# zhvng/open-musiclm

Measured on AMD Instinct MI355X. Metric: train steps/sec + AR tokens/sec, coarse-stage musiclm_small, higher is better.
Workload: dtype fp16ff; 1 GPU; musiclm_small coarse-stage train step (fwd+bwd+allreduce+clip+AdamW), N=1116 (3 start + 13 clap + 200 semantic + 900 coarse), forgetful mask 0.15, ff_dropout 0.1; global_batch=32, per_gpu_batch=32, grad_accum=1, seq_len=1116, parallelism=dp1, precision=fp16ff, hip_graph=True, exchange=none (single GPU)

## Files before the change

### include/omlm.h

```cpp
#ifndef OMLM_H
#define OMLM_H
#include <stdint.h>
#ifdef __cplusplus
extern "C" {
#endif

int         omlm_version(void);
const char* omlm_last_error(void);
void        omlm_set_error(const char* msg);

int omlm_gemm(const void* A, const void* B, void* C, const float* Cin,
              const int* a_map, const int* b_map, const int* c_map, long long a_rows, long long b_rows,
              int M, int N, int K, int lda, int ldb, int ldc, int ldcin,
              int a_kmajor, int b_kmajor, int in_dtype, int out_dtype, float alpha,
              void* workspace, long long workspace_bytes, void* stream);
long long omlm_gemm_tail_workspace_bytes(int M, int N);

int omlm_layernorm_fwd(const float* x, const float* gamma, void* y, void* xcast, float* mean, float* rstd,
                       int M, int D, int ldy, float eps, int out_dtype, void* stream);
int omlm_layernorm_fwd_planes(const float* x, const float* gamma, void* y, void* y_lo, float* mean, float* rstd,
                              int M, int D, int ldy, float eps, int out_dtype, void* stream);
int omlm_layernorm_fwd_seg(const float* x, const float* gamma, void* y, void* xcast, float* mean, float* rstd, float* xc,
                           int M, int D, int ldy, float eps, int out_dtype, int n_full, int p0, int n_live, void* stream);
int omlm_layernorm_fwd_planes_seg(const float* x, const float* gamma, void* y, void* y_lo, float* mean, float* rstd, float* xc,
                                  int M, int D, int ldy, float eps, int out_dtype, int n_full, int p0, int n_live, void* stream);
int omlm_layernorm_bwd2_seg(const void* dy, const float* x, const float* gamma, const float* mean, const float* rstd,
                            const float* dres, const void* dres2, float* dx, void* dxcast, float* dgamma, float* workspace, int M, int D,
                            float dx_scale, int cast_dtype, int dy_dtype, int n_full, int p0, int n_live, void* stream);
long long omlm_layernorm_bwd_workspace_bytes(int D);
int omlm_layernorm_bwd2(const void* dy, const float* x, const float* gamma, const float* mean, const float* rstd,
                        const float* dres, const void* dres2, float* dx, void* dxcast, float* dgamma, float* workspace, int M, int D,
                        float dx_scale, int cast_dtype, int dy_dtype, void* stream);

int omlm_qk_norm_fwd(const float* q_raw, const float* kv_raw, const float* q_scale, const float* k_scale,
                     void* q, void* k, void* v, int M, int H, int out_dtype, void* stream);
int omlm_qk_norm_bwd(const float* dq, const float* dk, const float* dv, const float* q_raw, const float* kv_raw,
                     const float* q_scale, const float* k_scale, void* dq_raw, void* dkv_raw,
                     float* dq_scale, float* dk_scale, int M, int H, int out_dtype, void* stream);

int omlm_gemm_qknorm(const void* A, const void* B, void* C, void* C2, int c2_col0, int ldc2, const float* scale, float* norm_out,
                     int ldnorm, int groups, long long a_rows, long long b_rows, int M, int N, int K, int lda, int ldb, int ldc,
                     int dtype, void* stream);
int omlm_qk_norm_bwd2(const float* dq, const float* dk, const float* dv, const void* q, const void* k, const float* qn, const float* kn,
                      const float* q_scale, const float* k_scale, void* dq_raw, void* dkv_raw, float* dq_scale, float* dk_scale,
                      int M, int H, int dtype, void* stream);

int omlm_mqa_attn_fwd(const void* q, const void* k, const void* v, const float* bias, const float* biasT, const unsigned char* keymask,
                      void* out, float* lse, int B, int N, int H, float scale, int bias_ld, int dtype, int P, float p,
                      unsigned long long seed, const unsigned long long* seed_dev, void* stream);
long long omlm_attn_bias_table_floats(int N, int H, int P);
int omlm_attn_bias_prepare(const float* bias, float* biasT, int N, int H, int bias_ld, const float* q_scale,
                           const float* k_scale, float qk_bound, float scale, int p_max_log2, void* stream);
int omlm_attn_bias_prepare_group(const float* bias, float* const* biasT, int layers, int N, int H, int bias_ld,
                                 const float* const* q_scale, const float* const* k_scale, float qk_bound, float scale,
                                 int p_max_log2, int P, void* stream);
int omlm_attn_max_positions(int dtype, int P);
long long omlm_mqa_attn_bwd_workspace_bytes(int B, int N, int H);
int omlm_mqa_attn_bwd(const void* q, const void* k, const void* v, const float* bias, const float* biasT, const unsigned char* keymask,
                      const void* out, const void* dout, const float* lse, float* delta, float* dq, float* dk, float* dv, float* dbias,
                      float* dbias_ws, int B, int N, int H, float scale, int bias_ld, int dtype, int P, float p, unsigned long long seed,
                      const unsigned long long* seed_dev, void* stream);
int omlm_attn_dropout_keep(unsigned char* keep, int B, int N, int H, float p, unsigned long long seed,
                           const unsigned long long* seed_dev, void* stream);
int omlm_dropout_residual_fwd(const float* x, const float* y, float* x1, long long M, int D, float p, unsigned long long seed,
                              const unsigned long long* seed_dev, void* stream);
int omlm_dropout_residual_bwd(const float* dx1, void* dy, long long M, int D, float p, unsigned long long seed,
                              const unsigned long long* seed_dev, int out_dtype, void* stream);

int omlm_ffmid_fwd(const void* h1, const void* convw, const void* gamma, void* h2, float* mean, float* rstd,
                   int M, int nseq, int F, int Fp, float eps, float p, unsigned long long seed,
                   const unsigned long long* seed_dev, unsigned char* drop_bits, void* gh, int dtype, void* stream);
int omlm_ffmid_fwd_planes(const void* h1, const void* h1_lo, const void* convw, const void* convw_lo, const void* gamma, const void* gamma_lo,
                          void* h2, void* h2_lo, float* mean, float* rstd, int M, int nseq, int F, int Fp, float eps, float p,
                          unsigned long long seed, const unsigned long long* seed_dev, unsigned char* drop_bits, void* gh, int dtype, void* stream);
int omlm_ffmid_fwd_seg(const void* h1, const void* convw, const void* gamma, void* h2, float* mean, float* rstd,
                       int M, int nseq, int F, int Fp, float eps, float p, unsigned long long seed,
                       const unsigned long long* seed_dev, unsigned char* drop_bits, void* gh, int dtype, int n_full, int p0, void* stream);
int omlm_ffmid_fwd_planes_seg(const void* h1, const void* h1_lo, const void* convw, const void* convw_lo, const void* gamma, const void* gamma_lo,
                              void* h2, void* h2_lo, float* mean, float* rstd, int M, int nseq, int F, int Fp, float eps, float p,
                              unsigned long long seed, const unsigned long long* seed_dev, unsigned char* drop_bits, void* gh, int dtype,
                              int n_full, int p0, void* stream);
long long omlm_ffmid_bwd_workspace_bytes(int F, int Fp);
int omlm_ffmid_bwd(const void* dh2, const void* h1, const void* convw, const void* gamma, const float* mean,
                   const float* rstd, void* du_tmp, void* dh1, float* dgamma, float* dconv, float* workspace,
                   int M, int nseq, int F, int Fp, float p, unsigned long long seed,
                   const unsigned long long* seed_dev, const unsigned char* drop_bits, const void* gh, int dtype, void* stream);
int omlm_colsum_accumulate(const float* part, float* out, int P, int C, int ldp, void* stream);
typedef struct omlm_colsum_desc { const float* part; float* out; int P, C, ldp; } omlm_colsum_desc;
int omlm_colsum_group(const omlm_colsum_desc* problems, int count, void* stream);
int omlm_ffmid_set_impl(int impl);

int omlm_embed_gather_fwd(const int* ids, const int* seg, const int* posidx,
                          const float* const* tables, const float* const* starts, const float* const* pos,
                          int nseq, float* out, int B, int N, int D,
                          const long long* table_rows, const long long* pos_rows, int* err_flag, void* stream);
int omlm_embed_gather_bwd(const int* ids, const int* seg, const int* posidx,
                          float* const* dtables, float* const* dstarts, float* const* dpos,
                          int nseq, const float* dx, int B, int N, int D, float alpha,
                          const long long* table_rows, const long long* pos_rows, int* err_flag, void* stream);

int omlm_prepare_train_batch(const long long* const* ids, int* const* labels, const int* len, const int* eos, const int* Q,
                             const int* codebook, int nseq, int B, int pad_id, const float* scores, int n_drop,
                             int* ids32, unsigned char* keymask, int N, const float* null_u, float null_p, void* stream);

int omlm_cross_entropy_fwd(const float* logits, const int* labels, float* row_lse, float* nll_sum,
                           int R, int V, int ld, int* err_flag, void* stream);
int omlm_cross_entropy_bwd(const float* logits, const int* labels, const float* row_lse, const float* gscale,
                           float coef, void* dlogits, int R, int V, int ld, int ldd, int out_dtype, void* stream);
int omlm_cross_entropy_fwd_reg(const float* logits, const int* labels, float* row_lse, float* sums,
                               int R, int V, int ld, int* err_flag, void* stream);
int omlm_cross_entropy_bwd_reg(const float* logits, const int* labels, const float* row_lse, const float* gscale,
                               float coef, void* dlogits, int R, int V, int ld, int ldd, int out_dtype,
                               float label_smoothing, float z_loss, void* stream);
int omlm_ce_metrics(const float* logits, const int* labels, float* row_nll, int* row_rank, float* row_entropy,
                    int R, int V, int ld, int* err_flag, void* stream);
// ... 177 lines not shown
```

### open_musiclm_amd/engine.py

```python
from __future__ import annotations

import math
import os
from dataclasses import dataclass, field
from typing import Dict, List, Optional, Sequence, Tuple

import torch

from . import ops
from .hip import require_gpu

ATTN_SCALE = 8.0
DIM_HEAD = 64

_PRECISIONS = {"bf16": torch.bfloat16, "bf16x3": torch.float32, "fp16": torch.float16, "fp16ff": torch.float16}


def is_half(precision: str) -> bool:
    return precision in ("fp16", "fp16ff")
_H16 = (torch.bfloat16, torch.float16)



FF_PLANES_MAX_FP = 4096
# ... 90 lines not shown

def build_layout(B: int, lens: Sequence[int], quantizers: Sequence[int], device, final_rows_only: bool = False) -> SeqLayout:
    starts, pos = [], 0
    for l in lens:
        starts.append(pos)
        pos += l + 1
    N = pos
    seg = torch.empty(N, dtype=torch.int32)
    posidx = torch.zeros(N, dtype=torch.int32)
    start_col = torch.zeros(N, dtype=torch.bool)
    for s, (st, l) in enumerate(zip(starts, lens)):
        seg[st: st + l + 1] = s
        start_col[st] = True
        posidx[st + 1: st + l + 1] = torch.arange(l, dtype=torch.int32)
    n_out = [l for l in lens[:-1]] + [lens[-1] + 1]
    lay = SeqLayout(B, N, tuple(lens), tuple(starts), tuple(n_out), seg.to(device), posidx.to(device),
                    start_col.to(device), final_rows_only)
    if final_rows_only:
        s, st, n_s, Q = len(lens) - 1, starts[-1], n_out[-1], quantizers[-1]
        b = torch.arange(B)
        a_map = (b * N + st + n_s - 1).to(torch.int32)
        lay.head_maps[(s, (n_s - 1) % Q)] = (a_map.to(device), b.to(torch.int32).to(device), B)
        return lay
    for s, (st, n_s, Q) in enumerate(zip(starts, n_out, quantizers)):
        for qq in range(Q):
            js = torch.arange(qq, n_s, Q)
            if js.numel() == 0:
                continue
            b = torch.arange(B)[:, None]
            a_map = (b * N + st + js[None, :]).reshape(-1).to(torch.int32)
            c_map = (b * n_s + js[None, :]).reshape(-1).to(torch.int32)
            lay.head_maps[(s, qq)] = (a_map.to(device), c_map.to(device), int(a_map.numel()))
    return lay


CONV_HALO = 2
LIVE_K_MULTIPLE = 64
FF_ONE_PASS_MAX_FP = 3072


def first_live_row(lay: SeqLayout, want: Sequence[bool]) -> Optional[int]:
    firsts = [st for st, n_s, w in zip(lay.starts, lay.n_out, want) if w and n_s > 0]
    return min(firsts) if firsts else None


def live_rows(lay: SeqLayout, want: Sequence[bool], B: int, T: torch.dtype, Fp: int, halo: int = CONV_HALO) -> Optional[Tuple[int, int, int]]:
    if os.environ.get("OMLM_LIVE_ROWS", "1") == "0":
        return None
    if lay.final_only or T == torch.float32 or Fp > FF_ONE_PASS_MAX_FP:
        return None
    first = first_live_row(lay, want)
    if first is None:
        return None
    N = lay.N
    g = LIVE_K_MULTIPLE // math.gcd(B, LIVE_K_MULTIPLE)
    top = first - halo
    if top < 0:
        return None
    p0 = top - (top - N) % g
    if p0 <= 0 or 16 * p0 < N:
        return None
    return N, p0, N - p0


def live_to_full(r, seg: Tuple[int, int, int]):
    n_full, p0, n_live = seg
    return (r // n_live) * n_full + p0 + r % n_live


def full_to_live(r, seg: Tuple[int, int, int]):
    n_full, p0, n_live = seg
    return (r // n_full) * n_live + r % n_full - p0


def head_map(lay: SeqLayout, s: int, qq: int, live: Optional[Tuple[int, int, int]]):
    ent = lay.head_maps.get((s, qq))
    if ent is None or live is None:
        return ent
    a_map, c_map, rows = ent
    key = (s, qq, live[1])
    if key not in lay.live_maps:
        lay.live_maps[key] = full_to_live(a_map, live).to(torch.int32)
    return lay.live_maps[key], c_map, rows


def h16_operand(w: torch.Tensor, T: torch.dtype) -> torch.Tensor:
    sh = getattr(w, "_omlm_bf16", None)
    if (sh is not None and sh.dtype == T and getattr(w, "_omlm_bf16_version", -1) == w._version and sh.device == w.device):
        return sh
    c = torch.empty(w.shape, dtype=T, device=w.device)
    ops.cast_pad(w.detach(), c, w.numel() // w.shape[-1], w.shape[-1], w.shape[-1], w.shape[-1])
    return c


class PreparedWeights:
    def __init__(self, model, precision: str, persistent: bool = True):
        tr = model.transformer
        self.precision = precision
        self.T = _PRECISIONS[precision]
        self.ff3 = precision == "fp16ff"
        T = self.T
        dev = model.start_tokens[0].device
        D = tr.dim
        Fp_all = {ceil_to(ff.inner_dim, 64) for _, _, ff in tr.layers}
        self.ff_planes = self.ff3 and all(ff_planes_ok(f) for f in Fp_all)
        self.mx = self.ff_planes and all(ff_mx_ok(D, f) for f in Fp_all)
        quants = ops.QuantRowsGroup()
        self.layers = []
        wbuf = model.__dict__.setdefault("_omlm_wbuf", {})
        packs = ops.CastPadGroup()
        for li, (attn, _, ff) in enumerate(tr.layers):
            F = ff.inner_dim
            Fp = ceil_to(F, 64)
            w1 = ff.w_in.weight
            w2 = ff.w_out.weight
            ent = {}
            if T == torch.float32:
                ent["Wq"], ent["Wkv"], ent["Wo"] = attn.to_q.weight, attn.to_kv.weight, attn.to_out[0].weight
            else:
                for name, w in (("Wq", attn.to_q.weight), ("Wkv", attn.to_kv.weight), ("Wo", attn.to_out[0].weight)):
                    ent[name] = h16_operand(w, T)
            bkey = (li, T, str(dev), F, D)
            if not persistent:
                W1p, W2p, convp, gammap = (torch.zeros(2 * Fp, D, dtype=T, device=dev), torch.zeros(D, Fp, dtype=T, device=dev),
                                           torch.zeros(3, 2 * Fp, dtype=T, device=dev), torch.zeros(Fp, dtype=T, device=dev))
            else:
                if bkey not in wbuf:
                    wbuf[bkey] = (torch.zeros(2 * Fp, D, dtype=T, device=dev), torch.zeros(D, Fp, dtype=T, device=dev),
                                  torch.zeros(3, 2 * Fp, dtype=T, device=dev), torch.zeros(Fp, dtype=T, device=dev))
                W1p, W2p, convp, gammap = wbuf[bkey]
            packs.add(w1.detach(), W1p, F, D, D, D)
            packs.add(w1.detach()[F:], W1p[Fp:], F, D, D, D)
            packs.add(w2.detach(), W2p, D, F, F, Fp)
            ent["W1p"], ent["W2p"], ent["F"], ent["Fp"] = W1p, W2p, F, Fp
            if self.ff_planes:
                lkey = bkey + ("lo",)
                if not persistent or lkey not in wbuf:
                    lo = (torch.zeros(2 * Fp, D, dtype=T, device=dev), torch.zeros(D, Fp, dtype=T, device=dev),
                          torch.zeros(3, 2 * Fp, dtype=T, device=dev), torch.zeros(Fp, dtype=T, device=dev))
                    if persistent:
                        wbuf[lkey] = lo
                else:
                    lo = wbuf[lkey]
                W1l, W2l, convl, gammal = lo
                if not (self.mx and persistent):
                    packs.add(w1.detach(), W1l, F, D, D, D, lo=True)
                    packs.add(w1.detach()[F:], W1l[Fp:], F, D, D, D, lo=True)
                    packs.add(w2.detach(), W2l, D, F, F, Fp, lo=True)
                ent["W1p_lo"], ent["W2p_lo"], ent["convw_lo"], ent["gamma_mid_lo"] = W1l, W2l, convl, gammal
            if self.mx:
                mkey = bkey + ("mx",)
                if not persistent or mkey not in wbuf:
                    m8 = (ops.Fp8Planes(2 * Fp, D, dev), ops.Fp8Planes(D, Fp, dev))
                    if persistent:
                        wbuf[mkey] = m8
                else:
                    m8 = wbuf[mkey]
                quants.add(w1.detach(), m8[0], 0, F, D, D)
                quants.add(w1.detach()[F:], m8[0], Fp, F, D, D)
                quants.add(w2.detach(), m8[1], 0, D, F, F)
                ent["W1p8"], ent["W2p8"] = m8
            cw = ff.conv_weight().detach().reshape(2 * F, 3)
            packs.add(cw, convp, F, 3, 3, 2 * Fp, transpose=True)
            packs.add(cw[F:], convp[:, Fp:], F, 3, 3, 2 * Fp, transpose=True)
            packs.add(ff.norm_mid.gamma.detach(), gammap, 1, F, F, Fp)
            ent["convw"], ent["gamma_mid"] = convp, gammap
# ... 153 lines not shown
    ops.gemm(dtable, lin[3].weight.detach(), dz, M=n, N=Hd, K=ldb, b_kmajor=True, lda=ldb, b_rows=H)
    for k in (2, 1):
        ds = torch.empty(n, Hd, device=dev)
        ops.silu_bwd(dz, pres[k], ds, n * Hd)
        ops.colsum_accumulate(ds, grad_of(lin[k].bias), n, Hd, Hd)
        gw = grad_of(lin[k].weight)
        ops.gemm(ds, zs[k - 1], gw, M=Hd, N=Hd, K=n, a_kmajor=True, b_kmajor=True, Cin=gw, planes=False)
        dz = torch.zeros(n, Hd, device=dev)
        ops.gemm(ds, lin[k].weight.detach(), dz, M=n, N=Hd, K=Hd, b_kmajor=True, Cin=dz, planes=False)
    ds = torch.empty(n, Hd, device=dev)
    ops.silu_bwd(dz, pres[0], ds, n * Hd)
    ops.colsum_accumulate(ds, grad_of(lin[0].bias), n, Hd, Hd)
    ops.relpos_first_bwd(ds, grad_of(lin[0].weight).view(-1), n, Hd, x0=x0)


class LayerSaved:
    __slots__ = ("x", "m1", "r1", "xn", "xc", "q_raw", "kv_raw", "q", "k", "v", "o", "lse", "abias",
                 "x1", "m2", "r2", "xn2", "h1", "h2", "m3", "r3", "seed", "p", "drop_bits", "gh", "h1_lo_tail",
                 "pa", "sa", "po", "so")


def _dropout_state(tr, dev):
    st = tr.__dict__.get("_omlm_dropout")
    if st is None or st["counter"].device != dev:
        rank = int(os.environ.get("RANK", "0"))
        g = torch.Generator().manual_seed((int(torch.initial_seed()) + 0x9E3779B1 * rank) & 0x7FFFFFFF)
        L = len(tr.layers)
        st = dict(counter=torch.zeros(1, dtype=torch.int64, device=dev),
                  seeds=[int(v) for v in torch.randint(1, 2 ** 62, (L,), generator=g)])
        a = [int(v) for v in torch.randint(1, 2 ** 62, (2 * L,), generator=g)]
        st["attn_seeds"], st["out_seeds"] = a[:L], a[L:]
        st["last"] = None
        tr.__dict__["_omlm_dropout"] = st
    return st


def dropout_salt(tr, dev) -> torch.Tensor:
    st = _dropout_state(tr, dev)
    st["counter"].add_(1)
    st["last"] = st["counter"].clone()
    return st["last"], st["seeds"]


def dropout_state(tr, dev=None) -> dict:
    st = tr.__dict__.get("_omlm_dropout")
    if st is None:
        st = _dropout_state(tr, dev if dev is not None else torch.device("cpu"))
    last = st["last"]
    return dict(ff=list(st["seeds"]), attn=list(st["attn_seeds"]), out=list(st["out_seeds"]),
                salt=int(last.item()) if last is not None else None)


def trunk_forward(tr, pw: PreparedWeights, x: torch.Tensor, keymask: Optional[torch.Tensor], B: int, N: int,
                  save: bool, training: bool, keep_h1_lo_tail: bool = False, live: Optional[Tuple[int, int, int]] = None):
    T = pw.T
    dev = x.device
    M, D = x.shape
    H = tr.heads
    P = prefix_rows(tr)
    rc = tr.__dict__.get("_omlm_relpos_cache")
    if rc is not None and save and training and rc.usable(N):
        table, rp_saved = rc.table, ("cached", rc)
    else:
        table, rp_saved = relpos_forward(tr, N, save, P)
        if (rc is not None and rc.enabled and rc.n is None and save and training and rp_saved is not None and rp_saved[0] != "t5"
                and not torch.cuda.is_current_stream_capturing()):
            rc.adopt(N, table, rp_saved)
            rp_saved = ("cached", rc)
    saved_layers: List[LayerSaved] = []
    abiases = None
    assert live is None or (len(tr.layers) > 0 and not keep_h1_lo_tail and live[0] == N)
    salt, seeds, aseeds, oseeds = (None, None, None, None)
    aps = [(float(a_.attn_dropout.p), float(a_.to_out[1].p)) if training else (0.0, 0.0) for a_, _, _ in tr.layers]
    if training and (any(float(ff.dropout_p) > 0 for _, _, ff in tr.layers) or any(pa > 0 or po > 0 for pa, po in aps)):
        salt, seeds = dropout_salt(tr, dev)
        st_ = tr.__dict__["_omlm_dropout"]
        aseeds, oseeds = st_["attn_seeds"], st_["out_seeds"]
    for li, ((attn, _, ff), w) in enumerate(zip(tr.layers, pw.layers)):
        sv = LayerSaved()
        F, Fp = w["F"], w["Fp"]
        m1 = torch.empty(M, device=dev); r1 = torch.empty(M, device=dev)
        xn = torch.empty(M, D, dtype=T, device=dev)
        xc = x if T == torch.float32 else torch.empty(M, D, dtype=T, device=dev)
        ops.layernorm_fwd(x, attn.norm.gamma.detach(), xn, None if T == torch.float32 else xc, m1, r1)
        q = torch.empty(M, H * DIM_HEAD, dtype=T, device=dev)
        k = torch.empty(M, DIM_HEAD, dtype=T, device=dev)
        v = torch.empty(M, DIM_HEAD, dtype=T, device=dev)
        fused_qk = T in _H16
        if fused_qk:
            qn = torch.empty(M, H, device=dev)
            kn = torch.empty(M, device=dev)
            q_raw, kv_raw = qn, kn
            ops.gemm_qknorm(xn, w["Wq"], q, attn.q_scale.detach(), qn, H, M=M, N=H * DIM_HEAD, K=D)
            ops.gemm_qknorm(xc, w["Wkv"], k, attn.k_scale.detach(), kn, 1, M=M, N=2 * DIM_HEAD, K=D, C2=v, c2_col0=DIM_HEAD)
        else:
            q_raw = torch.empty(M, H * DIM_HEAD, device=dev)
            kv_raw = torch.empty(M, 2 * DIM_HEAD, device=dev)
            ops.gemm(xn, w["Wq"], q_raw, M=M, N=H * DIM_HEAD, K=D)
            ops.gemm(xc, w["Wkv"], kv_raw, M=M, N=2 * DIM_HEAD, K=D)
            ops.qk_norm_fwd(q_raw, kv_raw, attn.q_scale.detach(), attn.k_scale.detach(), q, k, v, H)
        o = torch.empty(M, H * DIM_HEAD, dtype=T, device=dev)
        lse = torch.empty(B, H, N, device=dev)
        if abiases is None:
            abiases = ops.AttnBias.group(table, N, H, dev, [a_.q_scale.detach() for a_, _, _ in tr.layers],
                                         [a_.k_scale.detach() for a_, _, _ in tr.layers], scale=ATTN_SCALE, half=T == torch.float16, P=P)
        abias = abiases[li]
        pa, po = aps[li]
        sa = aseeds[li] if pa > 0 else 0
        so = oseeds[li] if po > 0 else 0
        ops.attn_fwd(q, k, v, abias, keymask, o, lse, B, N, H, ATTN_SCALE, P=P, p=pa, seed=sa, seed_dev=salt if pa > 0 else None)
        x1 = torch.empty(M, D, device=dev)
        if po > 0:
            yo = torch.empty(M, D, device=dev)
            ops.gemm(o, w["Wo"], yo, M=M, N=D, K=H * DIM_HEAD)
            ops.dropout_residual_fwd(x, yo, x1, po, so, seed_dev=salt)
            del yo
        else:
            ops.gemm(o, w["Wo"], x1, M=M, N=D, K=H * DIM_HEAD, Cin=x)
        seg = live if li == len(tr.layers) - 1 else None
        x1c = None
        if seg is not None:
            M = B * seg[2]
            nff = seg[2]
            x1c = torch.empty(M, D, device=dev)
        else:
            nff = N
        m2 = torch.empty(M, device=dev); r2 = torch.empty(M, device=dev)
        xn2 = torch.empty(M, D, dtype=T, device=dev)
        h1 = torch.empty(M, 2 * Fp, dtype=T, device=dev)
        if pw.mx:
            P1 = ops.Fp8Planes(M, D, dev, zero=False)
            ops.layernorm_fwd_mx(x1, ff.norm_in.gamma.detach(), xn2, P1, m2, r2, seg=seg, xc=x1c)
            h1_lo = torch.empty(M, 2 * Fp, dtype=torch.uint8, device=dev)
            ops.gemm_mx16(xn2, P1, w["W1p"], w["W1p8"], h1, h1_lo, M=M, N=2 * Fp, K=D)
        elif pw.ff_planes:
            xn2_lo = torch.empty(M, D, dtype=T, device=dev)
            ops.layernorm_fwd_planes(x1, ff.norm_in.gamma.detach(), xn2, xn2_lo, m2, r2, seg=seg, xc=x1c)
            h1_lo = torch.empty(M, 2 * Fp, dtype=T, device=dev)
            ops.gemm_planes16(xn2, xn2_lo, w["W1p"], w["W1p_lo"], h1, h1_lo, M=M, N=2 * Fp, K=D)
        else:
            ops.layernorm_fwd(x1, ff.norm_in.gamma.detach(), xn2, None, m2, r2, seg=seg, xc=x1c)
            ops.gemm(xn2, w["W1p"], h1, M=M, N=2 * Fp, K=D)
        if seg is not None:
            x1 = x1c
        h2 = torch.empty(M, Fp, dtype=T, device=dev)
        m3 = torch.empty(M, device=dev); r3 = torch.empty(M, device=dev)
        p = float(ff.dropout_p) if training else 0.0
        seed = seeds[li] if (p > 0 and seeds is not None) else 0
        drop_bits = torch.empty(M, Fp // 8, dtype=torch.uint8, device=dev) if (p > 0 and (save or pw.ff_planes)) else None
        gh = torch.empty(M, Fp, dtype=T, device=dev) if save else None
        x2 = torch.empty(M, D, device=dev)
        if pw.ff_planes:
            if pw.mx:
                P2 = ops.Fp8Planes(M, Fp, dev, zero=False)
                ops.ffmid_fwd_mx(h1, h1_lo, w["convw"], w["convw_lo"], w["gamma_mid"], w["gamma_mid_lo"], h2, P2, m3, r3, nff, F, Fp, p, seed,
                                 seed_dev=salt if p > 0 else None, drop_bits=drop_bits, gh=gh, seg=seg)
                ops.gemm_mx16(h2, P2, w["W2p"], w["W2p8"], x2, M=M, N=D, K=Fp, Cin=x1)
            else:
                h2_lo = torch.empty(M, Fp, dtype=T, device=dev)
                ops.ffmid_fwd_planes(h1, h1_lo, w["convw"], w["convw_lo"], w["gamma_mid"], w["gamma_mid_lo"], h2, h2_lo, m3, r3, nff, F, Fp, p, seed,
                                     seed_dev=salt if p > 0 else None, drop_bits=drop_bits, gh=gh, seg=seg)
                ops.gemm_planes16(h2, h2_lo, w["W2p"], w["W2p_lo"], x2, M=M, N=D, K=Fp, Cin=x1)
                del xn2_lo, h2_lo
            if keep_h1_lo_tail and save:
                take = min(2, N)
                sv.h1_lo_tail = torch.zeros(B, 2, 2 * Fp, device=dev)
                tail = h1_lo.view(B, N, -1)[:, N - take:]
                if tail.dtype == torch.uint8:
                    tail = (tail.contiguous().to(torch.int16) << 8).view(torch.float16)
                sv.h1_lo_tail[:, 2 - take:].copy_(tail)
            del h1_lo
        else:
            ops.ffmid_fwd(h1, w["convw"], w["gamma_mid"], h2, m3, r3, nff, F, Fp, p, seed, seed_dev=salt if p > 0 else None,
                          drop_bits=drop_bits, gh=gh, seg=seg)
            ops.gemm(h2, w["W2p"], x2, M=M, N=D, K=Fp, Cin=x1)
        if save:
            sv.x, sv.m1, sv.r1, sv.xn, sv.xc = x, m1, r1, xn, xc
# ... 409 lines not shown
```

### open_musiclm_amd/hip.py

```python
from __future__ import annotations

import ctypes as C
import os
from typing import Optional

import torch

_HERE = os.path.dirname(os.path.abspath(__file__))
LIB_PATH = os.environ.get("OMLM_LIB_PATH") or os.path.join(_HERE, "libomlm_hip.so")

_lib: Optional[C.CDLL] = None

vp, i32, i64, f32, u64, f64, u32 = C.c_void_p, C.c_int, C.c_longlong, C.c_float, C.c_ulonglong, C.c_double, C.c_uint

SIGNATURES = {
    "omlm_version": [],
    "omlm_last_error": [],
    "omlm_set_error": [C.c_char_p],
    "omlm_gemm": [vp, vp, vp, vp, vp, vp, vp, i64, i64, i32, i32, i32, i32, i32, i32, i32, i32, i32, i32, i32, f32, vp, i64, vp],
    "omlm_gemm_tail_workspace_bytes": [i32, i32],
    "omlm_gemm_wgrad_group": [vp, i32, i32, i32, vp],
    "omlm_gemm_planes": [vp, i64, vp, i64, vp, vp, vp, vp, vp, i64, i64, i32, i32, i32, i32, i32, i32, i32, i32, i32, i32, f32, vp, i64, vp],
    "omlm_split_planes": [vp, vp, i64, i64, vp],
    "omlm_gemm_planes16": [vp, vp, vp, vp, vp, vp, vp, vp, vp, i64, i64, i32, i32, i32, i32, i32, i32, i32, i32, vp, i64, vp],
    "omlm_gemm_mx16": [vp, vp, i64, vp, vp, vp, i64, vp, vp, vp, i32, vp, i64, i64, i32, i32, i32, i32, i32, i32, i32, vp, i64, vp],
    "omlm_gemm_mx16_workspace_bytes": [i32, i32, i32],
    "omlm_layernorm_fwd_mx": [vp, vp, vp, vp, i64, vp, vp, vp, i32, i32, i32, f32, vp],
    "omlm_ffmid_fwd_mx": [vp, vp, vp, vp, vp, vp, vp, vp, i64, vp, vp, vp, i32, i32, i32, i32, f32, f32, u64, vp, vp, vp, vp],
    "omlm_layernorm_fwd_mx_seg": [vp, vp, vp, vp, i64, vp, vp, vp, vp, i32, i32, i32, f32, i32, i32, i32, vp],
    "omlm_ffmid_fwd_mx_seg": [vp, vp, vp, vp, vp, vp, vp, vp, i64, vp, vp, vp, i32, i32, i32, i32, f32, f32, u64, vp, vp, vp, i32, i32, vp],
    "omlm_quant_rows_mx": [vp, i32, vp],
    "omlm_layernorm_fwd_planes": [vp, vp, vp, vp, vp, vp, i32, i32, i32, f32, i32, vp],
    "omlm_ffmid_fwd_planes": [vp, vp, vp, vp, vp, vp, vp, vp, vp, vp, i32, i32, i32, i32, f32, f32, u64, vp, vp, vp, i32, vp],
    "omlm_layernorm_fwd": [vp, vp, vp, vp, vp, vp, i32, i32, i32, f32, i32, vp],
    "omlm_layernorm_fwd_seg": [vp, vp, vp, vp, vp, vp, vp, i32, i32, i32, f32, i32, i32, i32, i32, vp],
    "omlm_layernorm_fwd_planes_seg": [vp, vp, vp, vp, vp, vp, vp, i32, i32, i32, f32, i32, i32, i32, i32, vp],
    "omlm_layernorm_bwd2_seg": [vp, vp, vp, vp, vp, vp, vp, vp, vp, vp, vp, i32, i32, f32, i32, i32, i32, i32, i32, vp],
    "omlm_layernorm_bwd_workspace_bytes": [i32],
    "omlm_layernorm_bwd2": [vp, vp, vp, vp, vp, vp, vp, vp, vp, vp, vp, i32, i32, f32, i32, i32, vp],
    "omlm_qk_norm_fwd": [vp, vp, vp, vp, vp, vp, vp, i32, i32, i32, vp],
    "omlm_qk_norm_bwd": [vp, vp, vp, vp, vp, vp, vp, vp, vp, vp, vp, i32, i32, i32, vp],
    "omlm_gemm_qknorm": [vp, vp, vp, vp, i32, i32, vp, vp, i32, i32, i64, i64, i32, i32, i32, i32, i32, i32, i32, vp],
    "omlm_qk_norm_bwd2": [vp, vp, vp, vp, vp, vp, vp, vp, vp, vp, vp, vp, vp, i32, i32, i32, vp],
    "omlm_attn_bias_table_floats": [i32, i32, i32],
    "omlm_attn_bias_prepare": [vp, vp, i32, i32, i32, vp, vp, f32, f32, i32, vp],
    "omlm_attn_bias_prepare_group": [vp, vp, i32, i32, i32, i32, vp, vp, f32, f32, i32, i32, vp],
    "omlm_mqa_attn_fwd": [vp] * 8 + [i32, i32, i32, f32, i32, i32, i32, f32, u64, vp, vp],
    "omlm_mqa_attn_bwd": [vp] * 15 + [i32, i32, i32, f32, i32, i32, i32, f32, u64, vp, vp],
    "omlm_mqa_attn_bwd_workspace_bytes": [i32, i32, i32],
    "omlm_attn_max_positions": [i32, i32],
    "omlm_attn_dropout_keep": [vp, i32, i32, i32, f32, u64, vp, vp],
    "omlm_dropout_residual_fwd": [vp, vp, vp, i64, i32, f32, u64, vp, vp],
    "omlm_dropout_residual_bwd": [vp, vp, i64, i32, f32, u64, vp, i32, vp],
    "omlm_ffmid_fwd": [vp, vp, vp, vp, vp, vp, i32, i32, i32, i32, f32, f32, u64, vp, vp, vp, i32, vp],
    "omlm_ffmid_fwd_seg": [vp, vp, vp, vp, vp, vp, i32, i32, i32, i32, f32, f32, u64, vp, vp, vp, i32, i32, i32, vp],
    "omlm_ffmid_fwd_planes_seg": [vp, vp, vp, vp, vp, vp, vp, vp, vp, vp, i32, i32, i32, i32, f32, f32, u64, vp, vp, vp, i32, i32, i32, vp],
    "omlm_ffmid_bwd_workspace_bytes": [i32, i32],
    "omlm_ffmid_bwd": [vp, vp, vp, vp, vp, vp, vp, vp, vp, vp, vp, i32, i32, i32, i32, f32, u64, vp, vp, vp, i32, vp],
    "omlm_colsum_accumulate": [vp, vp, i32, i32, i32, vp],
    "omlm_colsum_group": [vp, i32, vp],
    "omlm_ffmid_set_impl": [i32],
    "omlm_embed_gather_fwd": [vp, vp, vp, vp, vp, vp, i32, vp, i32, i32, i32, vp, vp, vp, vp],
    "omlm_embed_gather_bwd": [vp, vp, vp, vp, vp, vp, i32, vp, i32, i32, i32, f32, vp, vp, vp, vp],
    "omlm_prepare_train_batch": [vp, vp, vp, vp, vp, vp, i32, i32, i32, vp, i32, vp, vp, i32, vp, f32, vp],
    "omlm_cross_entropy_fwd": [vp, vp, vp, vp, i32, i32, i32, vp, vp],
    "omlm_cross_entropy_bwd": [vp, vp, vp, vp, f32, vp, i32, i32, i32, i32, i32, vp],
    "omlm_cross_entropy_fwd_reg": [vp, vp, vp, vp, i32, i32, i32, vp, vp],
    "omlm_cross_entropy_bwd_reg": [vp, vp, vp, vp, f32, vp, i32, i32, i32, i32, i32, f32, f32, vp],
    "omlm_ce_metrics": [vp, vp, vp, vp, vp, i32, i32, i32, vp, vp],
    "omlm_ce_metrics_bins": [vp, vp, vp, vp, i32, i32, i32, i32, i32, vp, vp],
    "omlm_sumsq_accumulate": [vp, i64, vp, vp, vp],
    "omlm_adamw_clip_step": [vp, vp, vp, vp, vp, i64, f32, f32, f32, f32, f32, i32, f32, vp, f32, i32, i32, i32, vp, vp],
    "omlm_adamw_clip_step_ema": [vp, vp, vp, vp, vp, i64, f32, f32, f32, f32, f32, i32, f32, vp, f32, i32, i32, i32, vp, vp, f32, i32, i32, vp],
    "omlm_loss_scale_update": [vp, vp, f32, f32, i32, f32, f32, vp],
    "omlm_cast_pad": [vp, vp, i64, i32, i32, i32, i32, vp],
    "omlm_cast_pad_group": [vp, i32, i32, vp],
    "omlm_sample_topk_gumbel_at": [vp, vp, vp, vp, vp, i32, i32, i32, i32, f32, i32, vp],
    "omlm_sample_embed_at": [vp, vp, vp, vp, vp, i32, i32, i32, i32, f32, i32, vp, i64, i64, vp, i32, vp],
    "omlm_decode_step": [vp, vp, vp],
    "omlm_decode_advance": [vp, vp, vp],
    "omlm_relpos_first_fwd": [vp, vp, vp, vp, i32, i32, i32, vp],
    "omlm_relpos_first_bwd": [vp, vp, i32, i32, i32, vp],
    "omlm_bias_silu_fwd": [vp, vp, vp, vp, i64, i32, vp],
    "omlm_silu_bwd": [vp, vp, vp, i64, vp],
    "omlm_bias_add": [vp, vp, vp, i32, i32, i32, vp],
    "omlm_relpos_mlp_fwd": [vp] * 15 + [i32, i32, i32, i32, i32, vp],
    "omlm_relpos_mlp_bwd": [vp] * 19 + [i32, i32, i32, i32, i32, vp],
    "omlm_rvq_encode": [vp, vp, vp, vp, i32, i32, i32, i32, i32, vp],
    "omlm_nearest_centroid": [vp, vp, vp, i32, i32, i32, vp],
    "omlm_vq_accumulate": [vp, vp, i32, vp, vp, i32, i32, i32, vp],
    "omlm_vq_kmeans_update": [vp, vp, vp, vp, i32, i32, vp],
    "omlm_vq_ema_update": [vp, vp, vp, vp, vp, vp, vp, i32, i32, f32, f32, vp],
    "omlm_kmeans_pp_workspace_bytes": [i32, i32],
    "omlm_kmeans_pp_pick": [vp] * 9 + [i64, i32, i32, i32, i32, vp],
    "omlm_kmeans_pp_seed": [vp] * 9 + [i64, i32, i32, i32, i32, vp],
    "omlm_kmeans_minibatch_step": [vp] * 10 + [i32, i32, i32, i32, f64, f64, i32, vp],
    "omlm_kmeans_inertia": [vp, vp, vp, vp, i32, i32, i32, vp],
    "omlm_sample_topk_gumbel": [vp, vp, vp, i32, i32, i32, i32, f32, i32, vp],
    "omlm_sample_topk_gumbel_rng": [vp, u32, u32, i32, i32, vp, i32, i32, i32, i32, f32, i32, vp],
    "omlm_sample_topk_gumbel_at_rng": [vp, u32, u32, vp, i32, vp, vp, i32, i32, i32, i32, f32, i32, vp],
    "omlm_sample_embed_at_rng": [vp, u32, u32, vp, i32, vp, vp, i32, i32, i32, i32, f32, i32, vp, i64, i64, vp, i32, vp],
    "omlm_sample": [vp, vp],
    "omlm_sample_lp": [vp, vp, vp, vp],
    "omlm_sample_rows": [vp, vp, vp, vp, vp],
    "omlm_guide_logits": [vp, vp, vp, i32, i32, i32, f32, vp],
    "omlm_guide_logits_rows": [vp, vp, vp, i32, i32, i32, vp, vp],
    "omlm_decode_twin": [vp, vp, vp, vp, i32, i32, vp],
    "omlm_probe_tr16": [vp, vp],
}
_RESTYPES = {"omlm_last_error": C.c_char_p, "omlm_gemm_tail_workspace_bytes": C.c_longlong, "omlm_gemm_mx16_workspace_bytes": C.c_longlong, "omlm_ffmid_bwd_workspace_bytes": C.c_longlong,
             "omlm_attn_bias_table_floats": C.c_longlong, "omlm_mqa_attn_bwd_workspace_bytes": C.c_longlong,
             "omlm_layernorm_bwd_workspace_bytes": C.c_longlong, "omlm_kmeans_pp_workspace_bytes": C.c_longlong,
             "omlm_set_error": None}


class HipLibraryMissing(RuntimeError):
    pass


def lib() -> C.CDLL:
    global _lib
    if _lib is None:
# ... 40 lines not shown
```

### open_musiclm_amd/ops.py

```python
from __future__ import annotations

import ctypes as C
import os
import weakref
from typing import NamedTuple, Optional, Sequence

import torch

from . import hip
from .ema import check_ema_settings
from .hip import call, ptr, stream_ptr

F32, BF16, F16 = 0, 1, 2
_CODES = {torch.float32: F32, torch.bfloat16: BF16, torch.float16: F16}
H16 = (torch.bfloat16, torch.float16)


def dcode(dtype: torch.dtype) -> int:
    try:
        return _CODES[dtype]
    except KeyError:
        raise TypeError(f"unsupported operand dtype {dtype}") from None


# ... 214 lines not shown
    call("omlm_layernorm_fwd_planes", ptr(x), ptr(gamma), ptr(y), ptr(y_lo), ptr(mean), ptr(rstd),
         M, D, y.shape[-1], float(eps), dcode(y.dtype), stream_ptr())


def layernorm_fwd_mx(x, gamma, y, P: "Fp8Planes", mean, rstd, eps=1e-5, seg=None, xc=None):
    M, D = x.shape
    if seg is not None:
        M = _seg_rows(x, y, seg, xc)
        assert y.dtype == torch.float16 and P.ld == y.shape[-1] and P.rows >= M and mean.numel() == rstd.numel() == M
        call("omlm_layernorm_fwd_mx_seg", ptr(x), ptr(gamma), ptr(y), ptr(P.planes), P.stride, ptr(P.scale), ptr(mean), ptr(rstd), ptr(xc),
             M, D, y.shape[-1], float(eps), *seg, stream_ptr())
        return
    assert y.dtype == torch.float16 and P.ld == y.shape[-1] and P.rows >= M
    call("omlm_layernorm_fwd_mx", ptr(x), ptr(gamma), ptr(y), ptr(P.planes), P.stride, ptr(P.scale), ptr(mean), ptr(rstd),
         M, D, y.shape[-1], float(eps), stream_ptr())


class _QuantDesc(C.Structure):
    _fields_ = [("src", C.c_void_p), ("dst8", C.c_void_p), ("lo_stride", C.c_longlong), ("scale8", C.c_void_p),
                ("R", C.c_int), ("C", C.c_int), ("ld_src", C.c_int), ("ld8", C.c_int)]


class QuantRowsGroup(_DescGroup):
    desc, entry = _QuantDesc, "omlm_quant_rows_mx"

    def add(self, src, P: "Fp8Planes", row0: int, R: int, C_: int, ld_src: int):
        hip.require_gpu(src, "src")
        assert src.dtype == torch.float32 and row0 + R <= P.rows and C_ <= 2 * P.ld
        self.items.append((src, P, int(row0), int(R), int(C_), int(ld_src)))

    def _fields(self, item):
        src, P, row0, R, C_, ld_src = item
        pitch = 2 * P.ld
        return ptr(src), P.planes.data_ptr() + row0 * pitch, P.stride, P.scale.data_ptr() + row0, R, C_, ld_src, pitch


_LN_WS = {}
LN_BWD_PARTIAL_ROWS = 2048


def _ln_workspace(D: int, device) -> torch.Tensor:
    key = (D, str(device))
    if key not in _LN_WS:
        _LN_WS[key] = torch.empty(int(hip.lib().omlm_layernorm_bwd_workspace_bytes(D)) // 4, device=device)
    return _LN_WS[key]


class _ColsumDesc(C.Structure):
    _fields_ = [("part", C.c_void_p), ("out", C.c_void_p), ("P", C.c_int), ("C", C.c_int), ("ldp", C.c_int)]


class ColsumGroup(_DescGroup):
    desc, entry = _ColsumDesc, "omlm_colsum_group"

    def add(self, part: torch.Tensor, out: torch.Tensor, P: int, C_: int, ldp: int):
        self.items.append((part, out, int(P), int(C_), int(ldp)))


def layernorm_bwd(dy, x, gamma, mean, rstd, dres, dx, dxcast, dgamma, dx_scale=1.0, dres2=None, defer: Optional["ColsumGroup"] = None, seg=None):
    M, D = x.shape
    if seg is not None:
        n_full, p0, n_live = seg
        assert dres2 is None and M % n_live == 0 and p0 + n_live == n_full and dy.shape[0] == M
        assert dx.shape[0] == M // n_live * n_full and (dxcast is None or dxcast.shape[0] == dx.shape[0]) and (dres is None or dres.shape[0] == M)
    code = dcode(dxcast.dtype) if dxcast is not None else (dcode(dres2.dtype) if dres2 is not None else F32)
    assert dres2 is None or dcode(dres2.dtype) == code, "dres2 must have the cast type"
    deferred = dgamma is not None and defer is not None
    rows = min(M, LN_BWD_PARTIAL_ROWS)
    if deferred:
        ws = torch.empty(rows * D, device=x.device)
    else:
        ws = _ln_workspace(D, x.device) if dgamma is not None else None
    if seg is not None:
        call("omlm_layernorm_bwd2_seg", ptr(dy), ptr(x), ptr(gamma), ptr(mean), ptr(rstd), ptr(dres), None, ptr(dx),
             ptr(dxcast), ptr(None if deferred else dgamma), ptr(ws), M, D, float(dx_scale), dcode(dy.dtype) if dxcast is None else code,
             dcode(dy.dtype), *seg, stream_ptr())
    else:
        call("omlm_layernorm_bwd2", ptr(dy), ptr(x), ptr(gamma), ptr(mean), ptr(rstd), ptr(dres), ptr(dres2), ptr(dx),
             ptr(dxcast), ptr(None if deferred else dgamma), ptr(ws), M, D, float(dx_scale), code, dcode(dy.dtype), stream_ptr())
    if deferred:
        defer.add(ws, dgamma, rows, D, D)


def qk_norm_fwd(q_raw, kv_raw, q_scale, k_scale, q, k, v, H):
    call("omlm_qk_norm_fwd", ptr(q_raw), ptr(kv_raw), ptr(q_scale), ptr(k_scale), ptr(q), ptr(k), ptr(v),
         q_raw.shape[0], H, dcode(q.dtype), stream_ptr())


def qk_norm_bwd(dq, dk, dv, q_raw, kv_raw, q_scale, k_scale, dq_raw, dkv_raw, dq_scale, dk_scale, H):
    call("omlm_qk_norm_bwd", ptr(dq), ptr(dk), ptr(dv), ptr(q_raw), ptr(kv_raw), ptr(q_scale), ptr(k_scale),
         ptr(dq_raw), ptr(dkv_raw), ptr(dq_scale), ptr(dk_scale), q_raw.shape[0], H, dcode(dq_raw.dtype), stream_ptr())


_DBIAS_WS = {}
_DBIAS_RETIRED = []


def gemm_qknorm(A, B, C_, scale, norm_out, groups, *, M, N, K, C2=None, c2_col0=0):
    hip.require_gpu(A, "A")
    assert A.dtype in H16 and B.dtype == A.dtype and C_.dtype == A.dtype and norm_out.dtype == torch.float32 and scale.dtype == torch.float32
    assert C2 is None or C2.dtype == A.dtype
    call("omlm_gemm_qknorm", ptr(A), ptr(B), ptr(C_), ptr(C2), int(c2_col0), C2.shape[-1] if C2 is not None else 0, ptr(scale), ptr(norm_out),
         norm_out.shape[-1] if norm_out.dim() > 1 else 1, int(groups), A.numel() // A.shape[-1], B.numel() // B.shape[-1], M, N, K,
         A.shape[-1], B.shape[-1], C_.shape[-1], dcode(A.dtype), stream_ptr())


def qk_norm_bwd2(dq, dk, dv, q, k, qn, kn, q_scale, k_scale, dq_raw, dkv_raw, dq_scale, dk_scale, H):
    call("omlm_qk_norm_bwd2", ptr(dq), ptr(dk), ptr(dv), ptr(q), ptr(k), ptr(qn), ptr(kn), ptr(q_scale), ptr(k_scale),
         ptr(dq_raw), ptr(dkv_raw), ptr(dq_scale), ptr(dk_scale), q.shape[0], H, dcode(dq_raw.dtype), stream_ptr())


class AttnBias:

    def __init__(self, table: Optional[torch.Tensor], N: int, H: int, device=None, q_scale=None, k_scale=None,
                 qk_bound: float = 0.0, scale: float = 8.0, half: bool = False, _tableT: Optional[torch.Tensor] = None, _P: int = 0):
        self.table, self.N, self.H, self.P = table, N, H, _P
        dev = table.device if table is not None else device
        if _tableT is not None:
            self.tableT = _tableT
            return
        self.tableT = torch.empty(int(hip.lib().omlm_attn_bias_table_floats(N, H, 0)), device=dev)
        call("omlm_attn_bias_prepare", ptr(table), ptr(self.tableT), N, H, table.shape[-1] if table is not None else 0,
             ptr(q_scale), ptr(k_scale), float(qk_bound), float(scale), 15 if half else 0, stream_ptr())

    @staticmethod
    def group(table: Optional[torch.Tensor], N: int, H: int, device, q_scales, k_scales, scale: float = 8.0, half: bool = False, P: int = 0):
        L = len(q_scales)
        dev = table.device if table is not None else device
        buf = torch.empty(L, int(hip.lib().omlm_attn_bias_table_floats(N, H, P)), device=dev)
        outs = (C.c_void_p * L)(*[buf[l].data_ptr() for l in range(L)])
        qs = (C.c_void_p * L)(*[t.data_ptr() for t in q_scales])
        ks = (C.c_void_p * L)(*[t.data_ptr() for t in k_scales])
        for t in list(q_scales) + list(k_scales):
            hip.require_gpu(t, "scale")
        call("omlm_attn_bias_prepare_group", ptr(table), C.cast(outs, C.c_void_p), L, N, H, table.shape[-1] if table is not None else 0,
             C.cast(qs, C.c_void_p), C.cast(ks, C.c_void_p), 0.0, float(scale), 15 if half else 0, int(P), stream_ptr())
        return [AttnBias(table, N, H, dev, _tableT=buf[l], _P=P) for l in range(L)]


def _attn_tables(bias, N, H, P, device):
    if isinstance(bias, AttnBias):
        if bias.P != P:
            raise ValueError(f"attention with P = {P} handed an AttnBias prepared for P = {bias.P}")
        return bias.table, bias.tableT
    return bias, (AttnBias(bias, N, H, device).tableT if P == 0 else None)


def _dbias_workspace(B: int, N: int, H: int, device) -> torch.Tensor:
    n = int(hip.lib().omlm_mqa_attn_bwd_workspace_bytes(B, N, H)) // 4
    key = str(device)
    ws = _DBIAS_WS.get(key)
    if ws is None or ws.numel() < n:
        if ws is not None:
            _DBIAS_RETIRED.append(ws)
        ws = _DBIAS_WS[key] = torch.empty(n, device=device, dtype=torch.float32)
    return ws


def attn_max_positions(dtype, P: int = 0) -> int:
    return int(hip.lib().omlm_attn_max_positions(dcode(dtype), int(P)))


def _check_positions(what, N, dtype, P):
    if P == 0 and dtype in H16 and N > attn_max_positions(dtype, 0):
        raise RuntimeError(f"{what}: N = {N} positions per sample is past the limit of {attn_max_positions(dtype, 0)} "
                           f"(omlm_attn_max_positions) of causal attention with {dtype} operands")
# ... 687 lines not shown
```

Before: 1189 samples/s.

## Fuse attention layernorm with the KV projection and key normalization

Adds a HIP kernel that computes the pre-attention layernorm and, from the same LDS-resident fp16 rows, also computes the 128-wide KV projection with MFMA plus key l2-normalization and scaling. The engine uses it when D<=1024 and 16-bit precision, which removes the separate gemm_qknorm launch for Wkv and the re-read of xc. The trade-offs are that the KV GEMM now runs with a split-K reduction through LDS inside a 1024-thread block, and that Wkv is streamed from global memory for every tile.

Result: no change. 1193 samples/s, median of 6 (+0.3%).

```diff
diff --git a/include/omlm.h b/include/omlm.h
--- a/include/omlm.h
+++ b/include/omlm.h
@@ -31,6 +31,8 @@
 int omlm_layernorm_bwd2(const void* dy, const float* x, const float* gamma, const float* mean, const float* rstd,
                         const float* dres, const void* dres2, float* dx, void* dxcast, float* dgamma, float* workspace, int M, int D,
                         float dx_scale, int cast_dtype, int dy_dtype, void* stream);
+int omlm_layernorm_kv_fwd(const float* x, const float* gamma, void* y, void* xcast, float* mean, float* rstd, const void* wkv,
+                          const float* k_scale, void* k, void* v, float* kn, int M, int D, int ldy, float eps, int dtype, void* stream);
 
 int omlm_qk_norm_fwd(const float* q_raw, const float* kv_raw, const float* q_scale, const float* k_scale,
                      void* q, void* k, void* v, int M, int H, int out_dtype, void* stream);
diff --git a/open_musiclm_amd/csrc/ln_kv.hip b/open_musiclm_amd/csrc/ln_kv.hip
--- /dev/null
+++ b/open_musiclm_amd/csrc/ln_kv.hip
@@ -0,0 +1,174 @@
+#include "common.h"
+
+#define LNKV_THREADS 1024
+#define LNKV_ROWS 16
+#define LNKV_MAX_D 1024
+#define LNKV_GRID 256
+#define LNKV_KV 128
+static inline int ln_kv_grid(int M) {
+    const int tiles = (M + LNKV_ROWS - 1) / LNKV_ROWS;
+    return tiles < LNKV_GRID ? tiles : LNKV_GRID;
+}
+#define LNKV_SLICES 8
+#define LNKV_XPAD 8
+#define LNKV_PPAD 4
+struct LnKvFwdArgs {
+    const float *x, *gamma, *k_scale;
+    const void* wkv;
+    void *y, *xcast, *k, *v;
+    float *mean, *rstd, *kn;
+    int M, D, ldy;
+    float eps;
+    void* stream;
+};
+static inline size_t ln_kv_fwd_lds(int D) {
+    return (size_t)LNKV_SLICES * LNKV_ROWS * (LNKV_KV + LNKV_PPAD) * sizeof(float) + (size_t)D * sizeof(float) + (size_t)LNKV_ROWS * (D + LNKV_XPAD) * 2;
+}
+
+namespace OMLM_NS {
+
+template <bool FULL>
+__device__ __forceinline__ float ln_sq4(float a, float b, float c, float d) {
+#pragma clang fp contract(off)
+    if constexpr (FULL) return (a * a + b * b) + (c * c + d * d);
+    else return __builtin_fmaf(a, a, b * b) + __builtin_fmaf(c, c, d * d);
+}
+
+template <bool FULL>
+__global__ __launch_bounds__(LNKV_THREADS) void ln_kv_fwd_kernel(const float* __restrict__ x, const float* __restrict__ gamma, h16_t* __restrict__ y,
+                                                                 h16_t* __restrict__ xcast, float* __restrict__ mean, float* __restrict__ rstd,
+                                                                 const h16_t* __restrict__ wkv, const float* __restrict__ k_scale,
+                                                                 h16_t* __restrict__ ko, h16_t* __restrict__ vo, float* __restrict__ kn,
+                                                                 int M, int Drt, int ldy, float eps) {
+    extern __shared__ __attribute__((aligned(16))) float lnkv_lds[];
+    const int D = FULL ? LNKV_MAX_D : Drt, nv = D / 4, xpitch = D + LNKV_XPAD, nks = D / 32;
+    constexpr int PP = LNKV_KV + LNKV_PPAD;
+    const int lane = threadIdx.x & 63, wave = __builtin_amdgcn_readfirstlane(threadIdx.x >> 6), r16 = lane & 15, kq = lane >> 4;
+    float* part = lnkv_lds;
+    float* gs = part + LNKV_SLICES * LNKV_ROWS * PP;
+    h16_t* xt = (h16_t*)(gs + D);
+    for (int c = threadIdx.x; c < D; c += LNKV_THREADS) gs[c] = gamma[c];
+    const float2 ks = *(const float2*)(k_scale + 2 * (lane & 31));
+    const int half = wave >> 3, slice = wave & 7;
+    const int ntiles = (M + LNKV_ROWS - 1) / LNKV_ROWS;
+    auto request = [&](float4 (&xv)[4], int tile) {
+        const int r = tile * LNKV_ROWS + wave;
+        const size_t rc = (size_t)(r < M ? r : M - 1);
+#pragma unroll
+        for (int i = 0; i < 4; ++i) {
+            const int c = lane + 64 * i;
+            xv[i] = (FULL || c < nv) ? ((const float4*)(x + rc * D))[c] : make_float4(0.f, 0.f, 0.f, 0.f);
+        }
+    };
+    float4 xv[4];
+    request(xv, blockIdx.x);
+    __syncthreads();
+#pragma unroll 1
+    for (int tile = blockIdx.x; tile < ntiles; tile += gridDim.x) {
+        const int row = tile * LNKV_ROWS + wave;
+        const bool live = row < M;
+        float t = 0.f;
+#pragma unroll
+        for (int i = 0; i < 4; ++i) {
+            const int c = lane + 64 * i;
+            const float s = (FULL || c < nv) ? (xv[i].x + xv[i].y) + (xv[i].z + xv[i].w) : 0.f;
+            t += wave_sum(s);
+        }
+        const float mu = t / (float)D;
+        float u = 0.f;
+#pragma unroll
+        for (int i = 0; i < 4; ++i) {
+            const int c = lane + 64 * i;
+            const float a = xv[i].x - mu, b = xv[i].y - mu, cc = xv[i].z - mu, d = xv[i].w - mu;
+            const float q = (FULL || c < nv) ? ln_sq4<FULL>(a, b, cc, d) : 0.f;
+            u += wave_sum(q);
+        }
+        const float rs = rsqrtf(u / (float)D + eps);
+        if (live) { mean[row] = mu; rstd[row] = rs; }
+#pragma unroll
+        for (int i = 0; i < 4; ++i) {
+            const int c = lane + 64 * i;
+            if (FULL || c < nv) {
+                const float4 g = *(const float4*)(gs + 4 * c);
+                const float a = xv[i].x - mu, b = xv[i].y - mu, cc = xv[i].z - mu, d = xv[i].w - mu;
+                u32x2 o;
+                o[0] = pack_h16_rne(xv[i].x, xv[i].y);
+                o[1] = pack_h16_rne(xv[i].z, xv[i].w);
+                *(u32x2*)(xt + wave * xpitch + 4 * c) = o;
+                if (live) {
+                    store4_from_float(y + (size_t)row * ldy + 4 * c, a * rs * g.x, b * rs * g.y, cc * rs * g.z, d * rs * g.w);
+                    *(u32x2*)(xcast + (size_t)row * D + 4 * c) = o;
+                }
+            }
+        }
+        request(xv, tile + (int)gridDim.x);
+        __syncthreads();
+        f32x4 acc[4];
+#pragma unroll
+        for (int ct = 0; ct < 4; ++ct) { acc[ct][0] = 0.f; acc[ct][1] = 0.f; acc[ct][2] = 0.f; acc[ct][3] = 0.f; }
+#pragma unroll
+        for (int j = 0; j < 4; ++j) {
+            const int kst = slice + LNKV_SLICES * j;
+            if (FULL || kst < nks) {
+                const u32x4 b = *(const u32x4*)(xt + r16 * xpitch + 32 * kst + 8 * kq);
+#pragma unroll
+                for (int ct = 0; ct < 4; ++ct) {
+                    const u32x4 a = *(const u32x4*)(wkv + (size_t)(64 * half + 16 * ct + r16) * D + 32 * kst + 8 * kq);
+                    acc[ct] = OMLM_MFMA_16x16x32(__builtin_bit_cast(h16x8, a), __builtin_bit_cast(h16x8, b), acc[ct]);
+                }
+            }
+        }
+#pragma unroll
+        for (int ct = 0; ct < 4; ++ct)
+            *(float4*)(part + (slice * LNKV_ROWS + r16) * PP + 64 * half + 16 * ct + 4 * kq) = make_float4(acc[ct][0], acc[ct][1], acc[ct][2], acc[ct][3]);
+        __syncthreads();
+        float a = 0.f, b = 0.f;
+#pragma unroll
+        for (int sl = 0; sl < LNKV_SLICES; ++sl) {
+            const float2 p = *(const float2*)(part + (sl * LNKV_ROWS + wave) * PP + 2 * lane);
+            a += p.x; b += p.y;
+        }
+        const float ss = wave_sum(lane < 32 ? a * a + b * b : 0.f);
+        const float nrm = fmaxf(sqrtf(ss), 1e-12f), inv = 1.0f / nrm;
+        if (live) {
+            if (lane < 32) *(unsigned*)(ko + (size_t)row * 64 + 2 * lane) = pack_h16_rne(a * inv * ks.x, b * inv * ks.y);
+            else *(unsigned*)(vo + (size_t)row * 64 + 2 * (lane - 32)) = pack_h16_rne(a, b);
+            kn[row] = nrm;
+        }
+    }
+}
+
+static int ln_kv_fwd_here(const LnKvFwdArgs& a) {
+    const int grid = ln_kv_grid(a.M);
+    const size_t lds = ln_kv_fwd_lds(a.D);
+    const hipStream_t st = as_stream(a.stream);
+    auto go = [&](auto fl) {
+        constexpr bool FULL = decltype(fl)::value;
+        launch_lds_cap<ln_kv_fwd_kernel<FULL>>(dim3(grid), dim3(LNKV_THREADS), lds, st, a.x, a.gamma, (h16_t*)a.y, (h16_t*)a.xcast, a.mean, a.rstd,
+                                               (const h16_t*)a.wkv, a.k_scale, (h16_t*)a.k, (h16_t*)a.v, a.kn, a.M, a.D, a.ldy, a.eps);
+    };
+    if (a.D == LNKV_MAX_D) go(std::true_type()); else go(std::false_type());
+    return omlm_post_launch("omlm_layernorm_kv_fwd");
+}
+
+#if OMLM_FP16
+extern "C" __attribute__((visibility("hidden"))) int omlm_ln_kv_fwd_h(const LnKvFwdArgs* a) { return ln_kv_fwd_here(*a); }
+#else
+extern "C" int omlm_ln_kv_fwd_h(const LnKvFwdArgs* a);
+
+extern "C" int omlm_layernorm_kv_fwd(const float* x, const float* gamma, void* y, void* xcast, float* mean, float* rstd, const void* wkv,
+                                     const float* k_scale, void* k, void* v, float* kn, int M, int D, int ldy, float eps, int dtype, void* stream) {
+    OMLM_CHECK_ARG(dtype == OMLM_DT_BF16 || dtype == OMLM_DT_F16, "layernorm_kv_fwd: 16-bit operand types only (1 = bf16, 2 = fp16)");
+    OMLM_CHECK_ARG(D > 0 && D % 64 == 0 && D <= LNKV_MAX_D, "layernorm_kv_fwd: D must be a multiple of 64 and <= 1024");
+    OMLM_CHECK_ARG(ldy >= D && ldy % 4 == 0, "layernorm_kv_fwd: ldy");
+    if (M <= 0) return OMLM_OK;
+    OMLM_CHECK_ARG(x && gamma && y && xcast && mean && rstd && wkv && k_scale && k && v && kn, "null pointer");
+    LnKvFwdArgs a;
+    memset(&a, 0, sizeof(a));
+    a.x = x; a.gamma = gamma; a.k_scale = k_scale; a.wkv = wkv; a.y = y; a.xcast = xcast; a.k = k; a.v = v; a.mean = mean; a.rstd = rstd; a.kn = kn;
+    a.M = M; a.D = D; a.ldy = ldy; a.eps = eps; a.stream = stream;
+    return dtype == OMLM_DT_F16 ? omlm_ln_kv_fwd_h(&a) : ln_kv_fwd_here(a);
+}
+#endif
+
+}
diff --git a/open_musiclm_amd/engine.py b/open_musiclm_amd/engine.py
--- a/open_musiclm_amd/engine.py
+++ b/open_musiclm_amd/engine.py
@@ -196,6 +196,10 @@
     if key not in lay.live_maps:
         lay.live_maps[key] = full_to_live(a_map, live).to(torch.int32)
     return lay.live_maps[key], c_map, rows
+
+
+def kv_fold_route(T: torch.dtype, D: int, dim_head: int = DIM_HEAD) -> bool:
+    return ops.ln_kv_ok(T, D, dim_head)
 
 
 def h16_operand(w: torch.Tensor, T: torch.dtype) -> torch.Tensor:
@@ -515,17 +519,22 @@
         m1 = torch.empty(M, device=dev); r1 = torch.empty(M, device=dev)
         xn = torch.empty(M, D, dtype=T, device=dev)
         xc = x if T == torch.float32 else torch.empty(M, D, dtype=T, device=dev)
-        ops.layernorm_fwd(x, attn.norm.gamma.detach(), xn, None if T == torch.float32 else xc, m1, r1)
         q = torch.empty(M, H * DIM_HEAD, dtype=T, device=dev)
         k = torch.empty(M, DIM_HEAD, dtype=T, device=dev)
         v = torch.empty(M, DIM_HEAD, dtype=T, device=dev)
         fused_qk = T in _H16
+        fold = kv_fold_route(T, D)
+        kn = torch.empty(M, device=dev) if fused_qk else None
+        if fold:
+            ops.layernorm_kv_fwd(x, attn.norm.gamma.detach(), xn, xc, m1, r1, w["Wkv"], attn.k_scale.detach(), k, v, kn)
+        else:
+            ops.layernorm_fwd(x, attn.norm.gamma.detach(), xn, None if T == torch.float32 else xc, m1, r1)
         if fused_qk:
             qn = torch.empty(M, H, device=dev)
-            kn = torch.empty(M, device=dev)
             q_raw, kv_raw = qn, kn
             ops.gemm_qknorm(xn, w["Wq"], q, attn.q_scale.detach(), qn, H, M=M, N=H * DIM_HEAD, K=D)
-            ops.gemm_qknorm(xc, w["Wkv"], k, attn.k_scale.detach(), kn, 1, M=M, N=2 * DIM_HEAD, K=D, C2=v, c2_col0=DIM_HEAD)
+            if not fold:
+                ops.gemm_qknorm(xc, w["Wkv"], k, attn.k_scale.detach(), kn, 1, M=M, N=2 * DIM_HEAD, K=D, C2=v, c2_col0=DIM_HEAD)
         else:
             q_raw = torch.empty(M, H * DIM_HEAD, device=dev)
             kv_raw = torch.empty(M, 2 * DIM_HEAD, device=dev)
diff --git a/open_musiclm_amd/hip.py b/open_musiclm_amd/hip.py
--- a/open_musiclm_amd/hip.py
+++ b/open_musiclm_amd/hip.py
@@ -38,6 +38,7 @@
     "omlm_layernorm_bwd2_seg": [vp, vp, vp, vp, vp, vp, vp, vp, vp, vp, vp, i32, i32, f32, i32, i32, i32, i32, i32, vp],
     "omlm_layernorm_bwd_workspace_bytes": [i32],
     "omlm_layernorm_bwd2": [vp, vp, vp, vp, vp, vp, vp, vp, vp, vp, vp, i32, i32, f32, i32, i32, vp],
+    "omlm_layernorm_kv_fwd": [vp, vp, vp, vp, vp, vp, vp, vp, vp, vp, vp, i32, i32, i32, f32, i32, vp],
     "omlm_qk_norm_fwd": [vp, vp, vp, vp, vp, vp, vp, i32, i32, i32, vp],
     "omlm_qk_norm_bwd": [vp, vp, vp, vp, vp, vp, vp, vp, vp, vp, vp, i32, i32, i32, vp],
     "omlm_gemm_qknorm": [vp, vp, vp, vp, i32, i32, vp, vp, i32, i32, i64, i64, i32, i32, i32, i32, i32, i32, i32, vp],
diff --git a/open_musiclm_amd/ops.py b/open_musiclm_amd/ops.py
--- a/open_musiclm_amd/ops.py
+++ b/open_musiclm_amd/ops.py
@@ -320,6 +320,27 @@
         defer.add(ws, dgamma, rows, D, D)
 
 
+LN_KV_MAX_D = 1024
+LN_KV_WIDTH = 128
+
+
+def ln_kv_ok(dtype: torch.dtype, D: int, dim_head: int = 64) -> bool:
+    return dtype in H16 and int(dim_head) == 64 and 0 < int(D) <= LN_KV_MAX_D and int(D) % 64 == 0
+
+
+def layernorm_kv_fwd(x, gamma, y, xcast, mean, rstd, wkv, k_scale, k, v, kn, eps=1e-5):
+    M, D = x.shape
+    T = y.dtype
+    assert ln_kv_ok(T, D), (T, D)
+    assert xcast.dtype == T and wkv.dtype == T and k.dtype == T and v.dtype == T and kn.dtype == torch.float32 and k_scale.dtype == torch.float32
+    assert wkv.shape == (LN_KV_WIDTH, D) and xcast.shape == (M, D) and k.shape == (M, 64) and v.shape == (M, 64) and kn.numel() == M
+    assert mean.numel() == M and rstd.numel() == M and y.shape[0] == M
+    for t_, n_ in ((x, "x"), (y, "y"), (xcast, "xcast"), (wkv, "wkv"), (k, "k"), (v, "v"), (kn, "kn")):
+        _chk(t_, n_)
+    call("omlm_layernorm_kv_fwd", ptr(x), ptr(gamma), ptr(y), ptr(xcast), ptr(mean), ptr(rstd), ptr(wkv), ptr(k_scale), ptr(k), ptr(v), ptr(kn),
+         M, D, y.shape[-1], float(eps), dcode(T), stream_ptr())
+
+
 def qk_norm_fwd(q_raw, kv_raw, q_scale, k_scale, q, k, v, H):
     call("omlm_qk_norm_fwd", ptr(q_raw), ptr(kv_raw), ptr(q_scale), ptr(k_scale), ptr(q), ptr(k), ptr(v),
          q_raw.shape[0], H, dcode(q.dtype), stream_ptr())
```
